# Giovannibriglia/VectorizedBayesianNetwork

Measured on AMD Instinct MI355X. Metric: posterior queries/sec (infer_posterior, n_samples=1024) at 1/2/4/8 MI355X, higher is better.
Workload: dtype f32; 1 GPU; cfg4: 64node-kde10k-mcm; queries_per_gpu=4096, global_batch=4096, n_samples=1024, n_nodes=64, engine=monte_carlo_marginalization, parallelism=query-sharded dp1, gather=False, prune_barren=False, exact_f32=False, kde_distances=mfma, walk=plan-specialised (step table compiled in with hiprtc), plan_cache_hits=1, kde_moment_nodes=16

## Files before the change

### vectorizedbayesiannetwork_amd/csrc/vbn_walk_impl.h

```cpp
#pragma once
#ifndef __HIPCC_RTC__
#include <hip/hip_runtime.h>
#include <stdint.h>
#include <math.h>
#include <stdio.h>
#include <string.h>

#include <algorithm>
#endif

#include "vbn_hip_types.h"

#ifndef INFINITY
#define INFINITY __builtin_inff()
#endif

#define WAVE 64
#define KDE_CHUNKS 16
#define KDE_MT(st) ((st).reserved[7])
#define KDE_REC_TAIL 16
#define LOG_2PI_F 1.8378770664093453f

typedef float f32x16 __attribute__((ext_vector_type(16)));
typedef _Float16 f16x8 __attribute__((ext_vector_type(8)));
typedef _Float16 f16x2 __attribute__((ext_vector_type(2)));
typedef float f32x2 __attribute__((ext_vector_type(2)));
typedef float f32x4 __attribute__((ext_vector_type(4)));

#define OFF_W2H(st) ((st).reserved[0])


__device__ __forceinline__ void wave_sync() {
  __atomic_signal_fence(__ATOMIC_SEQ_CST);
  __builtin_amdgcn_wave_barrier();
  __atomic_signal_fence(__ATOMIC_SEQ_CST);
}

__device__ __forceinline__ float relu_nan(float x) { return __int_as_float(max(__float_as_int(x), 0)); }

template <int ACT>
__device__ __forceinline__ float act_fn(float x) {
  if (ACT == VBN_ACT_RELU) return relu_nan(x);
  if (ACT == VBN_ACT_TANH) return tanhf(x);
  if (ACT == VBN_ACT_GELU) return x * 0.5f * (1.0f + erff(x * 0.70710678118654752440f));
  return x > 0.f ? x : expm1f(x);
}

#define VBN_LN2_F 0.69314718055994530942f
__device__ __forceinline__ float log_hw(float x) { return __builtin_amdgcn_logf(x) * VBN_LN2_F; }

__device__ __forceinline__ float softplus_t(float x) {
#ifdef VBN_ABL_NOSOFTPLUS
  return x;
#endif
  if (x > 20.f) return x;
  const float e = __expf(x);
  if (x < -5.f) return e * (1.f - e * (0.5f - e * (0.33333334f - e * 0.25f)));
  const float u = 1.0f + e;
  return log_hw(u) * (e * __builtin_amdgcn_rcpf(u - 1.0f));
}

__device__ __forceinline__ uint2 philox2x32(uint2 c, uint32_t k) {
#pragma unroll
  for (int r = 0; r < 10; ++r) {
    const uint64_t p = (uint64_t)0xD256D193u * c.x;
    c = make_uint2(__builtin_amdgcn_bitop3_b32((uint32_t)(p >> 32), k, c.y, 0x96), (uint32_t)p);
    k += 0x9E3779B9u;
  }
  return c;
}

__device__ __forceinline__ float u01(uint32_t x) { return (float)(x >> 8) * (1.0f / 16777216.0f); }

__device__ __forceinline__ float bm_radius(float u1) {
  return __builtin_amdgcn_sqrtf(-2.0f * log_hw(u1));
}

__device__ __forceinline__ float box_muller(uint32_t a, uint32_t b) {
  const float u1 = (float)((a >> 8) + 1u) * (1.0f / 16777216.0f);
  const float u2 = (float)(b >> 8) * (1.0f / 16777216.0f);
  return bm_radius(u1) * __builtin_amdgcn_cosf(u2);
}

struct Lane {
  const float* P;
  const int32_t* ic;
  float* vals;
  float* scr;
  const float* wb;
  int lane;
  int64_t p;
  int64_t b;
  int s;
  int iter;
  bool valid;
  bool mirror;
  bool lean;
  bool noiseless;
  bool wq;
  mutable float bm_spare;
};

// ... 1188 lines not shown
template <class ARG>
__device__ __forceinline__ int kde_scan(const float4* __restrict__ rec, const float4* __restrict__ rev, int M,
                                        int j0, int j1, float rem, float csum, ARG arg) {
  const bool back = rem > 0.5f * csum;
  const float goal = back ? csum - rem : rem;
  const float lim = back ? float_below(goal) : goal;
  const float4* __restrict__ q = back ? rev + (M - j1) : rec + j0;
  const int n = j1 - j0;
  float cs = 0.f, c0 = 0.f, c1 = 0.f, c2 = 0.f, c3 = 0.f;
  int kt = n;
  float4 a0 = q[0], a1 = q[1], a2 = q[2], a3 = q[3];
  float4 b0 = q[4], b1 = q[5], b2 = q[6], b3 = q[7];
  for (int k = 0; k < n; k += 8) {
    {
      const float e0 = cs + __builtin_amdgcn_exp2f(arg(a0));
      const float e1 = e0 + __builtin_amdgcn_exp2f(arg(a1));
      const float e2 = e1 + __builtin_amdgcn_exp2f(arg(a2));
      const float e3 = e2 + __builtin_amdgcn_exp2f(arg(a3));
      if (e3 > lim) { c0 = e0; c1 = e1; c2 = e2; c3 = e3; kt = k; break; }
      cs = e3;
    }
    a0 = q[k + 8]; a1 = q[k + 9]; a2 = q[k + 10]; a3 = q[k + 11];
    if (k + 4 >= n) break;
    {
      const float e0 = cs + __builtin_amdgcn_exp2f(arg(b0));
      const float e1 = e0 + __builtin_amdgcn_exp2f(arg(b1));
      const float e2 = e1 + __builtin_amdgcn_exp2f(arg(b2));
      const float e3 = e2 + __builtin_amdgcn_exp2f(arg(b3));
      if (e3 > lim) { c0 = e0; c1 = e1; c2 = e2; c3 = e3; kt = k + 4; break; }
      cs = e3;
    }
    b0 = q[k + 12]; b1 = q[k + 13]; b2 = q[k + 14]; b3 = q[k + 15];
  }
  (void)c3;
  const int v = c0 > lim ? 0 : (c1 > lim ? 1 : (c2 > lim ? 2 : 3));
  const int kh = kt < n ? min(kt + v, n - 1) : n - 1;
  return min(max(back ? j1 - 1 - kh : j0 + kh, 0), M - 1);
}

#define KDE_MT_HEAD 8
#define KDE_MT_GROUP 8
__device__ __forceinline__ int kde_index_moments(const float* __restrict__ T, float xb0, float ucat,
                                                 const float4* __restrict__ rec, int M, float& total) {
  const cfloat* H = CP(T);
  const float u_lo = H[0], inv_d = H[1], dlt = H[2];
  const int n_cells = __float_as_int(H[3]), nch = __float_as_int(H[4]), per = __float_as_int(H[5]);
  const float gr = rintf((xb0 - u_lo) * inv_d);
  const bool in = gr >= 0.f && gr < (float)n_cells;
  if (!__all(in)) return -1;
  const float d = xb0 - fmaf(gr, dlt, u_lo);
  const int ng = (nch + KDE_MT_GROUP - 1) / KDE_MT_GROUP;
  const float4* __restrict__ row = reinterpret_cast<const float4*>(T + KDE_MT_HEAD) + (int)gr * (nch + ng + 1);
  auto poly = [&](const float4 c) { return fmaf(fmaf(fmaf(c.w, d, c.z), d, c.y), d, c.x); };
  total = poly(row[nch + ng]);
  const double thr = (double)ucat * (double)total;
  double cum = 0.0;
  float gs = 0.f;
  int g = ng - 1;
  bool hit = false;
  for (int k = 0; k < ng; ++k) {
    gs = poly(row[nch + k]);
    const double nx = cum + (double)gs;
    if (nx > thr) { g = k; hit = true; break; }
    cum = nx;
  }
  if (!hit) cum -= (double)gs;
  const int c1 = min(nch, (g + 1) * KDE_MT_GROUP);
  int ch = c1 - 1;
  float cs = 0.f;
  hit = false;
  for (int c = g * KDE_MT_GROUP; c < c1; ++c) {
    cs = poly(row[c]);
    const double nx = cum + (double)cs;
    if (nx > thr) { ch = c; hit = true; break; }
    cum = nx;
  }
  if (!hit) cum -= (double)cs;
  const int j0 = min(M, ch * per), j1 = min(M, j0 + per);
  const float4* __restrict__ rev = rec + (((M + 15) >> 4) * 16 + KDE_REC_TAIL);
  return kde_scan(rec, rev, M, j0, j1, (float)(thr - cum), cs,
                  [&](const float4 r) { return fmaf(r.y, -1.f, fmaf(r.x, xb0, -0.f)); });
}

__device__ __forceinline__ int kde_index_mfma(const vbn_walk_args& A, const vbn_step& st, const Lane& L,
                                              float ucat, float c_p, float& lsp) {
  const int M = st.k, nf = st.aux0, lane = L.lane;
  const int cb = kde_cb(M);
  int slots[4] = {0, 0, 0, 0};
  float scl[4] = {c_p, c_p, c_p, c_p};
  for (int f = 0; f < nf; ++f) slots[f] = L.ic[st.in_off + f];
  double tot = 0.0;
  float xv[4] = {0.f, 0.f, 0.f, 0.f};
  const float negsq = kde_own(L, slots, scl, nf, xv);
  const bool pre = (st.flags & VBN_F_PRECOMP) != 0;
  const float4* __restrict__ rec = reinterpret_cast<const float4*>(L.P + st.reserved[3]) + 4;
  if (nf == 1 && KDE_MT(st) >= 0 && !(st.flags & (VBN_F_PRECOMP | VBN_F_PRE_OUT)) &&
      __all(-negsq <= KDE_FFORM_MAX)) {
    float mtot = 0.f;
    const int idx = kde_index_moments(L.P + KDE_MT(st), 2.f * xv[0], ucat, rec, M, mtot);
    if (idx >= 0) {
      if (mtot > 0.f) lsp = __logf(mtot) + negsq * VBN_LN2_F;
      wave_sync();
      return idx;
    }
  }
  float shift = 0.f;
  bool halves = false;
#ifndef VBN_ABL_NOHALVES
  float hs[KDE_CHUNKS * (KDE_NSUB - 1)];
#endif
  if (pre) {
    if (st.flags & VBN_F_PRECOMP_Q) {
      const cfloat* q = precomp_qrow(A, st, L);
      for (int ch = 0; ch < KDE_CHUNKS; ++ch) {
        const float cs = q[ch];
        L.scr[ch * WAVE + lane] = cs;
        tot += (double)cs;
      }
      shift = q[KDE_CHUNKS];
    } else {
      const float* __restrict__ q = precomp_row(A, st, L);
      for (int ch = 0; ch < KDE_CHUNKS; ++ch) {
        const float cs = q[ch];
        L.scr[ch * WAVE + lane] = cs;
        tot += (double)cs;
      }
      shift = q[KDE_CHUNKS];
    }
  } else
#ifdef VBN_ABL_NOP1
  if (true) {
    for (int ch = 0; ch < KDE_CHUNKS; ++ch) { L.scr[ch * WAVE + lane] = 1.f; tot += 1.0; }
  } else
#endif
  {
    const bf16x8* __restrict__ pa = reinterpret_cast<const bf16x8*>(L.P + st.reserved[1]) + lane;
    const bool fform = __all(-negsq <= KDE_FFORM_MAX);
    shift = fform ? 0.f : -negsq;
#ifndef VBN_ABL_NOHALVES
    float* hsp = ((st.flags & VBN_F_PRE_OUT) || (cb >> 1) < KDE_HALF_MIN) ? nullptr : hs;
    halves = hsp != nullptr;
#else
    float* hsp = nullptr;
#endif
    if (nf == 1)
      tot = kde_pass1<1, 1>(pa, cb >> 1, L, slots, scl, nf, fform, hsp);
    else if (nf == 2 && fform)
      tot = kde_pass1<1, 2>(pa, cb >> 1, L, slots, scl, nf, fform, hsp);
    else
      tot = kde_pass1<2, 2>(pa, cb >> 1, L, slots, scl, nf, fform, hsp);
  }
  const int nfr = nf;
  const float xb0 = 2.f * xv[0], xb1 = 2.f * xv[1], xb2 = 2.f * xv[2];
  if (!pre && !(tot >= (double)kde_tiny(M))) {
    halves = false;
    float amax = -INFINITY;
    for (int j = 0; j < M; ++j) amax = fmaxf(amax, kde_arg_rec(rec[j], xb0, xb1, xb2, 0.f, nfr));
    shift = amax;
    tot = 0.0;
    for (int ch = 0; ch < KDE_CHUNKS; ++ch) {
      const int j0 = min(M, ch * cb * 16), j1 = min(M, j0 + cb * 16);
      float cs = 0.f;
      for (int j = j0; j < j1; ++j)
        cs += __builtin_amdgcn_exp2f(kde_arg_rec(rec[j], xb0, xb1, xb2, 0.f, nfr) - shift);
      L.scr[ch * WAVE + lane] = cs;
      tot += (double)cs;
    }
  }
  if (tot > 0.0) lsp = __logf((float)tot) + (shift + negsq) * VBN_LN2_F;
  if (st.flags & VBN_F_PRE_OUT) {
    for (int c = 0; c < KDE_CHUNKS; ++c) vwrite(L, st.out_col + c, L.scr[c * WAVE + lane]);
    vwrite(L, st.out_col + KDE_CHUNKS, shift);
    wave_sync();
    return -1;
  }
  const double thr = (double)ucat * tot;
  double cum = 0.0;
  int ch = KDE_CHUNKS - 1;
  for (int c2 = 0; c2 < KDE_CHUNKS; ++c2) {
    const double nx = cum + (double)L.scr[c2 * WAVE + lane];
    if (nx > thr) { ch = c2; break; }
    cum = nx;
  }
  const int j0 = min(M, ch * cb * 16), j1 = min(M, j0 + cb * 16);
#ifdef VBN_ABL_NOSCAN
  wave_sync();
  return min(j0, M - 1);
#endif
  float rem = (float)(thr - cum);
  float csum = L.scr[ch * WAVE + lane];
  int jlo = j0, jhi = j1;
#ifndef VBN_ABL_NOHALVES
  if (halves) {
    const double rd = thr - cum;
    float plo = 0.f, phi = csum;
    int klo = 0, khi = KDE_NSUB;
#pragma unroll
    for (int k = 1; k < KDE_NSUB; ++k) {
      const float pk = hs[ch * (KDE_NSUB - 1) + k - 1];
      if (rd >= (double)pk) { klo = k; plo = pk; }
      else if (khi == KDE_NSUB) { khi = k; phi = pk; }
    }
    const int cb32 = cb >> 1;
    jlo = klo ? min(M, j0 + 32 * kde_sub_blocks(cb32, klo)) : j0;
    jhi = khi < KDE_NSUB ? min(M, j0 + 32 * kde_sub_blocks(cb32, khi)) : j1;
    rem = (float)(rd - (double)plo);
    csum = phi - plo;
  }
#endif
  const float4* __restrict__ rev = rec + (((M + 15) >> 4) * 16 + KDE_REC_TAIL);
  int idx;
  const float nsh = -shift;
  if (nfr == 1)
    idx = kde_scan(rec, rev, M, jlo, jhi, rem, csum,
                   [&](const float4 r) { return fmaf(r.y, -1.f, fmaf(r.x, xb0, nsh)); });
  else if (nfr == 2)
    idx = kde_scan(rec, rev, M, jlo, jhi, rem, csum, [&](const float4 r) {
      return fmaf(r.z, -1.f, fmaf(r.y, xb1, fmaf(r.x, xb0, nsh)));
    });
  else
    idx = kde_scan(rec, rev, M, jlo, jhi, rem, csum, [&](const float4 r) {
      return fmaf(r.w, -1.f, fmaf(r.z, xb2, fmaf(r.y, xb1, fmaf(r.x, xb0, nsh))));
    });
  wave_sync();
  return idx;
}

__device__ __forceinline__ bool kde_logp_mfma(const vbn_step& st, const Lane& L, bool root, float c_p,
                                              float c_y, float cy, float log_n, float& lp, float lsp) {
  const int M = st.k, dp = st.aux0, D = st.out_dim, lane = L.lane;
  const int nb32 = min((KDE_CHUNKS * kde_cb(M)) >> 1, (((M + 31) >> 5) + KDE_PF - 1) / KDE_PF * KDE_PF);
  int slots[4] = {0, 0, 0, 0};
  float scl[4] = {c_p, c_p, c_p, c_p};
  for (int f = 0; f < dp; ++f) slots[f] = L.ic[st.in_off + f];
  for (int d = 0; d < D; ++d) { slots[dp + d] = st.out_col + d; scl[dp + d] = c_y; }
  const int ny = dp + D;
  float xv[4];
  const float sq_y = -kde_own(L, slots, scl, ny, xv);
  const float sq_p = root ? 0.f : -kde_own(L, slots, scl, dp, xv);
  const bool fform = __all(sq_y <= KDE_FFORM_MAX);
  const bf16x8* __restrict__ pay = reinterpret_cast<const bf16x8*>(L.P + st.reserved[2]) + lane;
  const float sy = kde_sums_nf(pay, nb32, L, slots, scl, ny, fform);
  constexpr float LN2 = 0.69314718055994531f;
#ifndef VBN_ABL_NOLSP
  if (!root && __all(lsp == lsp)) {
    wave_sync();
    if (!(sy >= kde_tiny(M))) return false;
    lp += ((__logf(sy) - (fform ? sq_y * LN2 : 0.f)) - lsp) + cy;
    return true;
  }
#endif
  float sp = 1.f;
  if (!root) {
    const bf16x8* __restrict__ pa = reinterpret_cast<const bf16x8*>(L.P + st.reserved[1]) + lane;
    sp = kde_sums_nf(pa, nb32, L, slots, scl, dp, fform);
  }
  wave_sync();
  if (!(sy >= kde_tiny(M)) || !(sp >= kde_tiny(M))) return false;
  const float corr = fform ? (root ? sq_y : sq_y - sq_p) * LN2 : 0.f;
  lp += root ? ((__logf(sy) - corr) + cy - log_n) : (((__logf(sy) - __logf(sp)) - corr) + cy);
  return true;
}

__device__ __forceinline__ int kde_csz(int M) { return (((M + KDE_CHUNKS - 1) / KDE_CHUNKS) + 7) & ~7; }

template <int NF>
__device__ __forceinline__ float kde_arg_valu(const float (&xv)[4], const float4 r) {
#pragma clang fp contract(off)
  const float d0 = xv[0] - r.x;
  float a = d0 * d0;
  if (NF > 1) { const float d1 = xv[1] - r.y; a = fmaf(d1, d1, a); }
  if (NF > 2) { const float d2 = xv[2] - r.z; a = fmaf(d2, d2, a); }
  return -a;
}

template <int NF>
__device__ __forceinline__ int kde_index_valu(const vbn_walk_args& A, const vbn_step& st, const Lane& L,
                                              float ucat, float c_p) {
#pragma clang fp contract(off)
  const float* __restrict__ kv = L.P + st.reserved[4];
  const int M = st.k, lane = L.lane, csz = kde_csz(M);
  float xv[4] = {0.f, 0.f, 0.f, 0.f};
// ... 434 lines not shown
```

### vectorizedbayesiannetwork_amd/plan.py

```python
from __future__ import annotations

import hashlib
import math
import os
from dataclasses import dataclass
from typing import Dict, List, Optional, Sequence, Tuple

import numpy as np
import torch
import torch.nn.functional as F

from .model import BNModel, CPDRecord

KIND_ID = {"gaussian_nn": 0, "linear_gaussian": 1, "mdn": 2, "kde": 3, "softmax_nn": 4, "categorical_table": 5}
KIND_MASK_TABLE = 1024
ROLE_SKIP, ROLE_LATENT, ROLE_FIXED, ROLE_PARAMS, ROLE_SELECT, ROLE_COLLECT = 0, 1, 2, 3, 4, 5
F_LOGP, F_ROOT, F_SHARED, F_STANDARDIZE, F_CLIP, F_F32L2, F_KDE_VALU = 1, 2, 4, 8, 16, 32, 64
F_KEEP, F_LPRESET, F_BM_FIRST, F_BM_SECOND, F_MLP_GENERIC = 128, 256, 512, 1024, 2048
ACT_ID = {"relu": 0, "tanh": 1, "gelu": 2, "elu": 3}
WITHIN_ID = {"uniform": 0, "triangular": 1, "gaussian": 2}
MODE_MCM, MODE_WEIGHTED, MODE_SAMPLE, MODE_GIBBS = 0, 1, 2, 3
STEP_INTS = 32
(S_KIND, S_ROLE, S_FLAGS, S_ACT, S_NIN, S_INOFF, S_OUTCOL, S_OUTDIM, S_FIXEDCOL, S_K, S_NOUT,
 S_NODEID, S_NOISE, S_AUX0, S_AUX1, S_AUX2, S_OFF_STD, S_OFF_W1, S_OFF_W2, S_OFF_B2, S_OFF_W3,
# ... 118 lines not shown
    csz = ((m + KDE_CHUNKS - 1) // KDE_CHUNKS + 7) & ~7
    a = np.full((KDE_CHUNKS * csz, nf), 1e15, np.float32)
    a[:m] = y
    return a.reshape(-1, 8, nf).transpose(0, 2, 1)


KDE_MOMENTS = os.environ.get("VBN_KDE_MOMENTS", "1") != "0"
KDE_MT_TERMS = 4
KDE_MT_Z = 0.028
KDE_MT_CHUNKS = 64
KDE_MT_MAX_CELLS = 16384
KDE_MT_EXP_MAX = 100.0
KDE_MT_EXP_MIN = -80.0
KDE_MT_HEADER = 8


def kde_moment_cells(y: np.ndarray):
    y = np.asarray(y, np.float32).reshape(-1)
    y64 = y.astype(np.float64)
    sq = (y64 * y64).astype(np.float32).astype(np.float64)
    ymax_abs = float(np.abs(y64).max())
    span = float(y64.max() - y64.min())
    w = max(span, 2.0)
    lo, hi = 2.0 * (float(y64.min()) - w), 2.0 * (float(y64.max()) + w)
    if ymax_abs == 0.0:
        delta = hi - lo
    else:
        delta = 2.0 * KDE_MT_Z / (math.log(2.0) * ymax_abs)
    delta32 = np.float32(delta)
    lo32 = np.float32(lo)
    n = int(math.ceil((hi - lo) / float(delta32))) + 1
    if n > KDE_MT_MAX_CELLS:
        return None
    centres = kde_moment_centres(lo32, delta32, n)
    e_max = np.max(centres[:, None] * y64[None, :] - sq[None, :], axis=1)
    if e_max.max() > KDE_MT_EXP_MAX or e_max.min() < KDE_MT_EXP_MIN:
        return None
    return lo32, delta32, np.float32(1.0 / float(delta32)), n


def kde_moment_centres(lo32, delta32, n: int) -> np.ndarray:
    g = np.arange(n, dtype=np.float64)
    return (g * np.float64(delta32) + np.float64(lo32)).astype(np.float32).astype(np.float64)


def kde_moment_chunks(m: int) -> Tuple[int, int]:
    per = -(-m // KDE_MT_CHUNKS)
    return -(-m // per), per


KDE_MT_GROUP = 8


def kde_moment_rows(n_chunks: int) -> int:
    return n_chunks + -(-n_chunks // KDE_MT_GROUP) + 1


def kde_moment_table(y: np.ndarray) -> Optional[np.ndarray]:
    cells = kde_moment_cells(y)
    if cells is None:
        return None
    lo32, delta32, inv32, n = cells
    y64 = np.asarray(y, np.float32).reshape(-1).astype(np.float64)
    sq = (y64 * y64).astype(np.float32).astype(np.float64)
    m = y64.size
    nch, per = kde_moment_chunks(m)
    centres = kde_moment_centres(lo32, delta32, n)
    pw = np.stack([(math.log(2.0) * y64) ** k / math.factorial(k) for k in range(KDE_MT_TERMS)], axis=1)
    ng = -(-nch // KDE_MT_GROUP)
    tab = np.zeros((n, kde_moment_rows(nch), KDE_MT_TERMS), np.float64)
    for j0 in range(0, m, 4096):
        j1 = min(m, j0 + 4096)
        wts = np.exp2(centres[:, None] * y64[None, j0:j1] - sq[None, j0:j1])
        contrib = wts[:, :, None] * pw[None, j0:j1, :]
        chunk = np.arange(j0, j1) // per
        for c in np.unique(chunk):
            tab[:, c, :] += contrib[:, chunk == c, :].sum(axis=1)
    for g in range(ng):
        tab[:, nch + g, :] = tab[:, g * KDE_MT_GROUP:min(nch, (g + 1) * KDE_MT_GROUP), :].sum(axis=1)
    tab[:, nch + ng, :] = tab[:, :nch, :].sum(axis=1)
    head = np.zeros(KDE_MT_HEADER, np.float32)
    head[:3] = [lo32, inv32, delta32]
    head[3:6] = np.array([n, nch, per], np.int32).view(np.float32)
    return np.concatenate([head, tab.astype(np.float32).reshape(-1)])


def _np(t: torch.Tensor) -> np.ndarray:
    return t.detach().to("cpu", torch.float32).numpy()


def _pack_mlp_generic(blob: _Blob, layers, offs: Dict[str, int]) -> Dict[str, int]:
    lane = np.arange(64)
    table = [len(layers)]
    for w, b in layers:
        w, b = _np(w), _np(b)
        out, nin = w.shape
        nblk, t1 = -(-out // 32), -(-nin // 2)
        wz = np.zeros((nblk * 32, 2 * t1), np.float32)
        wz[:out, :nin] = w
        frag = np.stack([np.stack([wz[32 * k + (lane & 31), 2 * t + (lane >> 5)] for t in range(t1)])
                         for k in range(nblk)])
        bz = np.zeros(nblk * 32, np.float32)
        bz[:out] = b
        bias = np.stack([bz[32 * k + _ROWS] for k in range(nblk)])
        table += [nin, out, blob.add(frag), blob.add(bias)]
    offs["w2"] = blob.add(np.asarray(table, np.int32).view(np.float32))
    offs["n_out"] = int(_np(layers[-1][0]).shape[0])
    offs["generic"] = 1
    offs["scratch"] = offs["n_out"] + 2 * max([int(w.shape[0]) for w, _ in layers[:-1]] + [1])
    return offs


def _pack_mlp(blob: _Blob, rec: CPDRecord, standardize: bool) -> Dict[str, int]:
    layers = rec.mlp_layers()
    hidden = tuple(int(w.shape[0]) for w, _ in layers[:-1])
    offs: Dict[str, int] = {}
    if standardize:
        inv = (np.float32(1.0) / _np(rec.state["std_x"]).astype(np.float32)).astype(np.float32)
        offs["std"] = blob.add(np.concatenate([_np(rec.state["mean_x"]), inv]))
    else:
        offs["std"] = 0
    if hidden != MLP_HIDDEN:
        return _pack_mlp_generic(blob, layers, offs)
    (w1, b1), (w2, b2), (w3, b3) = [(_np(w), _np(b)) for w, b in layers]
    nin = w1.shape[1]
    t1 = (nin + 1) // 2
    w1z = np.zeros((32, 2 * t1), np.float32)
    w1z[:, :nin] = w1
    lane = np.arange(64)
    w1f = np.stack([w1z[lane & 31, 2 * t + (lane >> 5)] for t in range(t1)])
    w2f = np.zeros((16, 64), np.float32)
    for s in range(16):
        w2f[s] = w2[lane & 31, _ROWS[lane >> 5, s]]
    offs["w1"] = blob.add(w1f)
    offs["wblk"] = offs["w1"]
    offs["b2"] = blob.add(np.stack([np.stack([b[_ROWS]] * 2) for b in (b1, b2)]))
    offs["f32l2"] = int(np.abs(w2).max() > 32768.0)
    rs = float(np.abs(w1.astype(np.float64)).sum(axis=1).max()) if w1.size else 0.0
    lim = 2048.0 if str(rec.hp("activation") or "relu") == "relu" else 32768.0
    room = lim * (1.0 - 1e-3) - float(np.abs(b1.astype(np.float64)).max())
    if room <= 1.0:
        offs["zlim"] = -1.0
    else:
        offs["zlim"] = float(np.float32(min(room / rs, 3.0e38))) if rs > 0 else 3.0e38
    j = np.arange(8)
    j3 = j
    frag = np.zeros((2, 64, 8), np.float32)
    for s in range(2):
        for ln in range(64):
            frag[s, ln] = w2[ln & 31, 16 * s + 8 * (j >> 2) + 4 * (ln >> 5) + (j & 3)]
    with np.errstate(over="ignore", invalid="ignore"):
        hi = frag.astype(np.float16)
        lo = (frag - hi.astype(np.float32)).astype(np.float16)
    halfs = np.concatenate([hi, lo]).reshape(-1)
    offs["w2h"] = blob.add(halfs.view(np.float32))
    offs["w3"] = blob.add(np.concatenate([w3[:, _ROWS[0]], w3[:, _ROWS[1]]], axis=1))
    offs["b3"] = blob.add(b3)
    n_out = w3.shape[0]
    if HEAD_MFMA_MIN <= n_out <= 32 and np.abs(w3).max() <= 32768.0:
        w3p = np.zeros((32, 32), np.float32)
        w3p[:n_out] = w3
        f3 = np.zeros((2, 64, 8), np.float32)
        for s_ in range(2):
            for ln in range(64):
                f3[s_, ln] = w3p[ln & 31, 16 * s_ + 8 * (j3 >> 2) + 4 * (ln >> 5) + (j3 & 3)]
        hi3 = f3.astype(np.float16)
# ... 57 lines not shown
    scratch: int = 0


def _pack_node(blob: _Blob, rec: CPDRecord) -> NodePack:
    kind = rec.kind
    D = rec.output_dim
    root = rec.is_root
    flags = F_ROOT if root else 0
    st = rec.state
    offs: Dict[str, int] = {}
    k = n_out = aux0 = aux1 = 0
    if kind == "categorical_table":
        offs = _pack_table(blob, rec)
        k, aux0, aux1 = offs.pop("_table")
        return NodePack(kind=KIND_ID[kind], flags=flags, act=0, n_in=rec.input_dim, out_dim=D, k=k, n_out=0,
                        aux0=aux0, aux1=aux1, offs=offs, scratch=0)
    act = ACT_ID.get(str(rec.hp("activation") or "relu"), -1)
    if act < 0:
        raise ValueError(f"unknown activation {rec.hp('activation')}")
    if kind == "gaussian_nn":
        if root:
            loc = st["_loc"].view(1, 1, -1)
            scale = (F.softplus(st["_log_scale"]) + float(rec.hp("min_scale"))).view(1, 1, -1)
            std_y = st["std_y"].view(1, 1, -1)
            loc, scale = loc * std_y + st["mean_y"].view(1, 1, -1), scale * std_y
            loc, scale = loc.reshape(-1), scale.reshape(-1)
            offs["tail"] = blob.add(np.concatenate([_np(loc), _np(scale), _np(scale.log())]))
        else:
            flags |= F_STANDARDIZE
            offs.update(_pack_mlp(blob, rec, standardize=True))
            n_out = offs.pop("n_out")
            offs["tail"] = blob.add(np.concatenate([_np(st["std_y"]), _np(st["mean_y"]),
                                                    np.array([rec.hp("min_scale")], np.float32)]))
    elif kind == "linear_gaussian":
        var = st["_var"]
        scale = torch.sqrt(var.clamp(min=float(rec.hp("min_scale")) ** 2))
        w = st["_weight"]
        offs["tail"] = blob.add(np.concatenate([_np(w.t().contiguous()).reshape(-1), _np(st["_bias"]),
                                                _np(scale), _np(torch.log(scale))]))
    elif kind == "mdn":
        k = int(rec.hp("n_components"))
        if root:
            pi = torch.softmax(st["_logits"], dim=-1).clamp_min(1e-5)
            pi = pi / pi.sum(dim=-1, keepdim=True).clamp_min(1e-12)
            scale = F.softplus(st["_log_scale"]) + float(rec.hp("min_scale"))
            log_scale = torch.log(scale)
            offs["tail"] = blob.add(np.concatenate([
                _np(pi), _np(torch.log(pi)), _np(st["_loc"]).reshape(-1), _np(scale).reshape(-1),
                _np(log_scale).reshape(-1), _np(torch.exp(2 * log_scale)).reshape(-1),
                _np(torch.softmax(st["_logits"], dim=-1))]))
        else:
            offs.update(_pack_mlp(blob, rec, standardize=False))
            n_out = offs.pop("n_out")
            if n_out != k * (2 * D) + k:
                raise ValueError("mdn head width mismatch")
            offs["tail"] = blob.add(np.array([rec.hp("min_scale")], np.float32))
    elif kind == "kde":
        pts_p = rec.extra["parents"].float()
        pts_y = rec.extra["targets"].float()
        m = int(pts_y.shape[0])
        dp = int(pts_p.shape[1]) if pts_p.dim() == 2 else 0
        if m == 0:
            raise RuntimeError("KDECPD is not fitted yet.")
        bw = float(rec.hp("bandwidth"))
        pbw = rec.hp("parent_bandwidth")
        pbw = bw if pbw is None else float(pbw)
        min_scale = float(rec.hp("min_scale"))
        s_p = max(pbw, 1e-3) + min_scale
        s_y = max(bw, 1e-3) + min_scale
        noise_scale = max(bw, 1e-3) + min_scale
        cy = -0.5 * D * (math.log(2 * math.pi) + 2 * math.log(s_y))
        c_p = np.float32(_KDE_C / s_p)
        c_y = np.float32(_KDE_C / s_y)
        offs["tail"] = blob.add(np.array([1.0 / np.float32(s_p), 1.0 / np.float32(s_y),
                                          noise_scale, cy, math.log(float(m)), c_p, c_y, 0], np.float32))
        if 1 <= dp <= 3:
            offs["kq"] = blob.add(_kde_pack_b32(_np(pts_p) * c_p))
            offs["kr"] = blob.add(_kde_pack([_np(pts_p) * c_p], records=True))
            offs["kv"] = blob.add(_kde_pack_valu(_np(pts_p) * c_p))
            if dp == 1 and KDE_MOMENTS:
                mt = kde_moment_table((_np(pts_p) * c_p).reshape(-1))
                if mt is not None:
                    offs["kmt"] = blob.add(mt)
        if dp + D <= 4:
            feats = np.concatenate(([_np(pts_p).reshape(m, -1) * c_p] if dp else [])
                                   + [_np(pts_y).reshape(m, -1) * c_y], axis=1)
            offs["kqy"] = blob.add(_kde_pack_b32(feats))
        stride = dp + D
        stride += (-stride) % 2 if stride > 1 else 0
        recs = np.zeros((m, stride), np.float32)
        if dp:
            recs[:, :dp] = _np(pts_p)
        recs[:, dp:dp + D] = _np(pts_y)
        offs["pts"] = blob.add(recs)
        k, aux0, aux1 = m, dp, stride
    elif kind == "softmax_nn":
        if str(rec.hp("mode_when_not_discrete") or "binned") != "binned":
            raise NotImplementedError("softmax_nn mode_when_not_discrete != 'binned'")
        if not bool(st["_bins_ready"]):
            raise RuntimeError("Bins not initialized. Call fit(...) before sampling.")
        k = int(rec.hp("n_classes"))
        aux0 = WITHIN_ID[str(rec.hp("within_bin"))]
        disc = st["_is_discrete"].bool()
        if D > 31:
            raise NotImplementedError("softmax_nn with more than 31 output dims")
        aux1 = int(sum(1 << d for d in range(D) if bool(disc[d])))
        if bool(rec.hp("within_bin_clip")):
            flags |= F_CLIP
        mbw = float(rec.hp("min_bin_width"))
        offs["tail"] = blob.add(np.concatenate([
            _np(st["_bin_edges"]).reshape(-1), _np(st["_sample_values"]).reshape(-1),
            _np(st["_class_values"]).reshape(-1),
            np.array([rec.hp("within_bin_scale"), mbw, mbw ** 2, 0.0], np.float32)]))
        if root:
            if bool(st["_root_ready"]):
                tab = torch.log_softmax(st["_root_log_probs"].view(D, k) / 1.0, dim=-1)
            else:
                tab = st["_logits"].view(D, k) / 1.0
            offs["pts"] = blob.add(_np(tab))
        else:
            offs.update(_pack_mlp(blob, rec, standardize=False))
            n_out = offs.pop("n_out")
    else:
        raise ValueError(kind)
    if offs.pop("generic", 0):
        flags |= F_MLP_GENERIC
    if offs.pop("f32l2", 0):
        flags |= F_F32L2
    scratch = offs.pop("scratch", n_out)
    return NodePack(kind=KIND_ID[kind], flags=flags, act=max(act, 0), n_in=rec.input_dim,
                    out_dim=D, k=k, n_out=n_out, aux0=aux0, aux1=aux1, offs=offs, scratch=scratch)


class PackedModel:

    def __init__(self, model: BNModel, device: torch.device):
        self.model = model
        self.device = torch.device(device)
        blob = _Blob()
        blob.add(np.zeros(4, np.float32))
        self.nodes: Dict[str, NodePack] = {}
        if len(model.topo) >= MAX_NODES:
            raise NotImplementedError(f"{len(model.topo)} nodes: the walk keys RNG streams for < {MAX_NODES}")
        for node in model.topo:
            if model.out_dim(node) >= MAX_NODE_DIMS:
                raise NotImplementedError(f"node {node}: {model.out_dim(node)} dims (max {MAX_NODE_DIMS - 1})")
            rec = model.cpds[node]
            expect = sum(model.out_dim(p) for p in model.parents[node])
            if rec.input_dim != expect:
                raise ValueError(f"node {node}: CPD input_dim {rec.input_dim} != parents width {expect}")
            self.nodes[node] = _pack_node(blob, rec)
        host = blob.finish()
        self.tabular = all(p.kind == KIND_ID["categorical_table"] for p in self.nodes.values())
        if self.tabular and host.size % WBLK_CHUNK:
            host = np.concatenate([host, np.zeros((-host.size) % WBLK_CHUNK, np.float32)])
        self.params = torch.from_numpy(host).to(self.device)
        self.node_id = {n: i for i, n in enumerate(model.topo)}
        self.max_out = max([p.scratch for p in self.nodes.values()] + [1])
        self.has_kde = any(p.kind == KIND_ID["kde"] for p in self.nodes.values())
        self.dmax = max(model.out_dim(n) for n in model.topo)


@dataclass
class QueryPlan:
    steps: torch.Tensor
    in_cols: torch.Tensor
# ... 129 lines not shown
    slot_of: Dict[str, int] = {}
    release: Dict[int, List[str]] = {}
    for i, n in enumerate(order):
        d = width(n)
        base = None
        if d == 1 and free:
            free.sort()
            base = free.pop(0)
        elif d > 1:
            fs = sorted(free)
            for j in range(len(fs) - d + 1):
                if fs[j + d - 1] - fs[j] == d - 1:
                    base = fs[j]
                    for q in range(d):
                        free.remove(base + q)
                    break
        if base is None:
            base = n_slots
            n_slots += d
        slot_of[n] = base
        release.setdefault(last[n], []).append(n)
        for m in release.pop(i, []):
            if m != n or last[n] == i:
                free.extend(range(slot_of[m], slot_of[m] + width(m)))
    fixed_nodes = [n for n in order if n in fixed_s]
    fixed_col = {}
    c = 0
    for n in fixed_nodes:
        fixed_col[n] = c
        c += model.out_dim(n)
    noise_nodes = [n for n in order if n in latent_s]
    noise_idx = {n: i for i, n in enumerate(noise_nodes)}
    steps = np.zeros((len(order), STEP_INTS), np.int32)
    in_cols: List[int] = []
    for i, n in enumerate(order):
        npk = packed.nodes[n]
        row = steps[i]
        row[S_KIND] = npk.kind
        row[S_ROLE] = ROLE_PARAMS if n in params_s else (ROLE_LATENT if n in latent_s else ROLE_FIXED)
        fl = npk.flags
        if n in logp_s:
            fl |= F_LOGP
        if shared_roots and (npk.flags & F_ROOT):
            fl |= F_SHARED
        if exact_f32:
            fl |= F_F32L2
        if kde_valu and npk.kind == KIND_ID["kde"]:
            fl |= F_KDE_VALU
        if n in pre_s:
            fl |= F_PRE_OUT
        if n in clamp_s and n in fixed_s:
            fl |= F_CLAMP_EV
        row[S_FLAGS] = fl
        row[S_ACT] = npk.act
        row[S_NIN] = npk.n_in
        row[S_INOFF] = len(in_cols)
        if reads[n]:
            for p in model.parents[n]:
                in_cols.extend(range(slot_of[p], slot_of[p] + model.out_dim(p)))
        row[S_OUTCOL] = slot_of[n]
        row[S_OUTDIM] = npk.out_dim
        row[S_FIXEDCOL] = fixed_col.get(n, 0)
        row[S_K] = npk.k
        row[S_NOUT] = npk.n_out
        row[S_NODEID] = packed.node_id[n]
        row[S_NOISE] = noise_idx.get(n, 0)
        row[S_AUX0] = npk.aux0
        row[S_AUX1] = npk.aux1
        for key, idx in (("std", S_OFF_STD), ("w1", S_OFF_W1), ("w2", S_OFF_W2), ("b2", S_OFF_B2),
                         ("w3", S_OFF_W3), ("b3", S_OFF_B3), ("tail", S_OFF_TAIL), ("pts", S_OFF_PTS),
                         ("w2h", S_OFF_W2H)):
            row[idx] = npk.offs.get(key, 0)
        row[S_OFF_KQ] = npk.offs.get("kq", -1)
        if "zlim" in npk.offs:
            row[S_OFF_KQ] = np.float32(npk.offs["zlim"]).view(np.int32)
        row[S_OFF_KQY] = npk.offs.get("kqy", -1)
        if "w3h" in npk.offs:
            row[S_OFF_KQY] = npk.offs["w3h"]
            fl |= F_HEAD_MFMA
            row[S_FLAGS] = fl
        row[S_OFF_KR] = npk.offs.get("kr", -1)
        row[S_OFF_KV] = npk.offs.get("kv", -1)
        row[S_RES7] = npk.offs.get("kmt", -1)
        if "wblk" in npk.offs and (n in latent_s or n in logp_s or n in params_s):
            row[S_WBLK_OFF] = npk.offs["wblk"]
            row[S_WBLK_LEN] = npk.offs["wblk_len"]
    out_cols: List[int] = []
    for n in out_nodes:
        out_cols.extend(range(slot_of[n], slot_of[n] + width(n)))
    dev = packed.device

    def t(a):
        a = np.asarray(a, np.int32).reshape(-1) if len(a) else np.zeros(1, np.int32)
        return torch.from_numpy(np.ascontiguousarray(a)).to(dev)

    _pair_normals(steps)
    kind_mask = 0
    for n in order:
        if n in latent_s or n in logp_s or n in params_s:
            npk = packed.nodes[n]
            kind_mask |= 1 << npk.kind
            if npk.n_out and npk.act != ACT_ID["relu"]:
                kind_mask |= 32
            if npk.flags & F_MLP_GENERIC:
                kind_mask |= 512
    tabular = bool(getattr(packed, "tabular", False))
    wbuf = int(steps[:, S_WBLK_LEN].max()) if len(order) else 0
    if tabular:
        kind_mask = KIND_MASK_TABLE
        wbuf = int(packed.params.numel())
        read_by = {p for n in order if reads[n] for p in model.parents[n]}
        table_check = [(n, fixed_col[n], n in clamp_s) for n in fixed_nodes
                       if n in logp_s or n in read_by or n in set(out_nodes)]
        cv_offs: List[int] = []
        for n in out_nodes:
            npk = packed.nodes[n]
            if n in params_s:
                cv_offs.extend([-1] * width(n))
            else:
                cv_offs.extend(npk.offs["w3"] + dd * npk.aux1 for dd in range(npk.out_dim))
    max_out = max([packed.nodes[n].scratch for n in order] + [1])
    if any(packed.nodes[n].kind == KIND_ID["kde"] for n in order):
        max_out = max(max_out, KDE_CHUNKS)
    steps_t = torch.from_numpy(steps).to(dev) if len(order) else torch.zeros(1, STEP_INTS, dtype=torch.int32, device=dev)
    steps_t._vbn_wblk_max = int(steps[:, S_WBLK_LEN].max()) if len(order) else 0
    ic_host = np.asarray(in_cols, np.int32).reshape(-1)
    steps_t._vbn_host = (steps.copy(), ic_host.copy(),
                         hashlib.sha1(steps.tobytes() + b"|" + ic_host.tobytes()).hexdigest())
    return QueryPlan(
        steps=steps_t,
        in_cols=t(in_cols), out_cols=t(out_cols), n_steps=len(order), n_slots=max(n_slots, 1),
        max_out=max_out, fixed_nodes=fixed_nodes, fixed_ld=max(c, 1), noise_nodes=noise_nodes,
        out_nodes=list(out_nodes), mode=mode, slot_of=slot_of, kind_mask=kind_mask, order=list(order),
        wbuf=wbuf, tabular=tabular, table_out_cols=t(out_cols + cv_offs) if tabular else None,
        table_check=table_check if tabular else None)


def _pair_normals(steps: np.ndarray) -> None:
    gauss = (KIND_ID["gaussian_nn"], KIND_ID["linear_gaussian"], KIND_ID["mdn"], KIND_ID["kde"])
    pending = -1
    for i in range(len(steps)):
        r = steps[i]
        if r[S_ROLE] != ROLE_LATENT or r[S_KIND] not in gauss or r[S_OUTDIM] != 1:
            continue
        if pending >= 0 and (steps[pending][S_FLAGS] & F_SHARED) == (r[S_FLAGS] & F_SHARED):
            steps[pending][S_FLAGS] |= F_BM_FIRST
            r[S_FLAGS] |= F_BM_SECOND
            pending = -1
        else:
            pending = i


@dataclass
class GibbsPlan:
    init: QueryPlan
    steps: torch.Tensor
    n_steps: int
    latent: List[str]
    target: str
    n_noise: int
    in_cols: torch.Tensor
    kind_mask: int
    wbuf: int = 0


def build_gibbs_plan(packed: PackedModel, *, latent: Sequence[str], fixed: Sequence[str], target: str,
# ... 350 lines not shown
```

Baseline: 55580 queries/s.

## Add 2D moment-table lookup for two-parent KDE chunk sums

Result: faster. 59770 queries/s, median of 6 (+7.5%).

```diff
diff --git a/vectorizedbayesiannetwork_amd/csrc/vbn_walk_impl.h b/vectorizedbayesiannetwork_amd/csrc/vbn_walk_impl.h
--- a/vectorizedbayesiannetwork_amd/csrc/vbn_walk_impl.h
+++ b/vectorizedbayesiannetwork_amd/csrc/vbn_walk_impl.h
@@ -18,6 +18,7 @@
 #define WAVE 64
 #define KDE_CHUNKS 16
 #define KDE_MT(st) ((st).reserved[7])
+#define KDE_MT2(st) ((st).off_w1)
 #define KDE_REC_TAIL 16
 #define LOG_2PI_F 1.8378770664093453f
 
@@ -1372,6 +1373,60 @@
                   [&](const float4 r) { return fmaf(r.y, -1.f, fmaf(r.x, xb0, -0.f)); });
 }
 
+#define KDE_MT2_HEAD 16
+#define KDE_MT2_K 9
+#define KDE_MT2_ROW4 12
+struct KdeMt2 {
+  const float4* cell;
+  float d0, d1;
+};
+
+__device__ __forceinline__ float kde_mt2_row(const float4* __restrict__ row, float d0, float d1) {
+  float4 v = row[0];
+  int i = 0;
+  auto next = [&]() {
+    const int k = i & 3;
+    if (i && !k) v = row[i >> 2];
+    ++i;
+    return k == 0 ? v.x : (k == 1 ? v.y : (k == 2 ? v.z : v.w));
+  };
+  float s = next();
+#pragma unroll
+  for (int a = KDE_MT2_K - 2; a >= 0; --a) {
+    float p = next();
+#pragma unroll
+    for (int b = KDE_MT2_K - 2 - a; b >= 0; --b) p = fmaf(p, d1, next());
+    s = fmaf(s, d0, p);
+  }
+  return s;
+}
+
+__device__ __noinline__ float kde_mt2_row_call(const float4* __restrict__ row, float d0, float d1) {
+  return kde_mt2_row(row, d0, d1);
+}
+
+__device__ __forceinline__ bool kde_index_moments2(const float* __restrict__ T, float u0, float u1, const Lane& L,
+                                                   bool halves, double& tot, KdeMt2& m) {
+  const cfloat* H = CP(T);
+  const float g0 = rintf((u0 - H[0]) * H[1]), g1 = rintf((u1 - H[4]) * H[5]);
+  const int n0 = __float_as_int(H[3]), n1 = __float_as_int(H[7]);
+  const bool in = g0 >= 0.f && g0 < (float)n0 && g1 >= 0.f && g1 < (float)n1;
+  if (!__all(in)) return false;
+  m.d0 = u0 - fmaf(g0, H[2], H[0]);
+  m.d1 = u1 - fmaf(g1, H[6], H[4]);
+  const int rows = halves ? 2 * KDE_CHUNKS : KDE_CHUNKS;
+  m.cell = reinterpret_cast<const float4*>(T + KDE_MT2_HEAD) + ((int)g0 * n1 + (int)g1) * (rows * KDE_MT2_ROW4);
+  double t = 0.0;
+#pragma unroll 1
+  for (int ch = 0; ch < KDE_CHUNKS; ++ch) {
+    const float cs = kde_mt2_row(m.cell + ch * KDE_MT2_ROW4, m.d0, m.d1);
+    L.scr[ch * WAVE + L.lane] = cs;
+    t += (double)cs;
+  }
+  tot = t;
+  return true;
+}
+
 __device__ __forceinline__ int kde_index_mfma(const vbn_walk_args& A, const vbn_step& st, const Lane& L,
                                               float ucat, float c_p, float& lsp) {
   const int M = st.k, nf = st.aux0, lane = L.lane;
@@ -1396,6 +1451,23 @@
   }
   float shift = 0.f;
   bool halves = false;
+  bool tab2 = false;
+  KdeMt2 mt2 = {nullptr, 0.f, 0.f};
+  if (nf == 2 && KDE_MT2(st) >= 0 && !(st.flags & (VBN_F_PRECOMP | VBN_F_PRE_OUT)) &&
+      __all(-negsq <= KDE_FFORM_MAX)) {
+#ifndef VBN_ABL_NOHALVES
+    const bool h2 = KDE_NSUB == 2 && (cb >> 1) >= KDE_HALF_MIN;
+#else
+    const bool h2 = false;
+#endif
+    double t2 = 0.0;
+    if (kde_index_moments2(L.P + KDE_MT2(st), 2.f * xv[0], 2.f * xv[1], L, (cb >> 1) >= KDE_HALF_MIN, t2, mt2) &&
+        __all(t2 >= (double)kde_tiny(M))) {
+      tab2 = true;
+      halves = h2;
+      tot = t2;
+    }
+  }
 #ifndef VBN_ABL_NOHALVES
   float hs[KDE_CHUNKS * (KDE_NSUB - 1)];
 #endif
@@ -1417,7 +1489,7 @@
       }
       shift = q[KDE_CHUNKS];
     }
-  } else
+  } else if (!tab2)
 #ifdef VBN_ABL_NOP1
   if (true) {
     for (int ch = 0; ch < KDE_CHUNKS; ++ch) { L.scr[ch * WAVE + lane] = 1.f; tot += 1.0; }
@@ -1487,7 +1559,8 @@
     int klo = 0, khi = KDE_NSUB;
 #pragma unroll
     for (int k = 1; k < KDE_NSUB; ++k) {
-      const float pk = hs[ch * (KDE_NSUB - 1) + k - 1];
+      const float pk = tab2 ? kde_mt2_row_call(mt2.cell + (KDE_CHUNKS + ch) * KDE_MT2_ROW4, mt2.d0, mt2.d1)
+                            : hs[ch * (KDE_NSUB - 1) + k - 1];
       if (rd >= (double)pk) { klo = k; plo = pk; }
       else if (khi == KDE_NSUB) { khi = k; phi = pk; }
     }
diff --git a/vectorizedbayesiannetwork_amd/plan.py b/vectorizedbayesiannetwork_amd/plan.py
--- a/vectorizedbayesiannetwork_amd/plan.py
+++ b/vectorizedbayesiannetwork_amd/plan.py
@@ -224,6 +224,95 @@
     head = np.zeros(KDE_MT_HEADER, np.float32)
     head[:3] = [lo32, inv32, delta32]
     head[3:6] = np.array([n, nch, per], np.int32).view(np.float32)
+    return np.concatenate([head, tab.astype(np.float32).reshape(-1)])
+
+
+KDE_MOMENTS2 = os.environ.get("VBN_KDE_MOMENTS2", "1") != "0"
+KDE_MT2_Z = 0.5
+KDE_MT2_K = 9
+KDE_MT2_COEFS = KDE_MT2_K * (KDE_MT2_K + 1) // 2
+KDE_MT2_ROW = (KDE_MT2_COEFS + 3) & ~3
+KDE_MT2_HEADER = 16
+KDE_MT2_MAX_BYTES = 32 << 20
+KDE_MT2_MARGINS = (2.0, 1.5, 1.0)
+KDE_HALF_MIN = 16
+
+
+def kde_moment2_order(k: int = KDE_MT2_K) -> List[Tuple[int, int]]:
+    return [(a, b) for a in range(k - 1, -1, -1) for b in range(k - 1 - a, -1, -1)]
+
+
+def kde_moment2_geometry(m: int) -> Tuple[int, int, bool]:
+    cb = _kde_cb(m)
+    cb32 = cb // 2
+    return 16 * cb, 32 * ((cb32 // 2) & ~1), cb32 >= KDE_HALF_MIN
+
+
+def kde_moment2_cells(y: np.ndarray, z: float = KDE_MT2_Z, w: float = KDE_MT2_MARGINS[0]):
+    y64 = np.asarray(y, np.float32).reshape(-1, 2).astype(np.float64)
+    out = []
+    for f in range(2):
+        c = y64[:, f]
+        lo, hi = 2.0 * (float(c.min()) - w), 2.0 * (float(c.max()) + w)
+        amax = float(np.abs(c).max())
+        delta32 = np.float32(hi - lo if amax == 0.0 else z / (math.log(2.0) * amax))
+        lo32 = np.float32(lo)
+        n = int(math.ceil((hi - lo) / float(delta32))) + 1
+        out.append((lo32, delta32, np.float32(1.0 / float(delta32)), n))
+    return out
+
+
+def kde_moment_table2(y: np.ndarray, z: float = KDE_MT2_Z, k: int = KDE_MT2_K) -> Optional[np.ndarray]:
+    y32 = np.asarray(y, np.float32).reshape(-1, 2)
+    m = y32.shape[0]
+    per, half, halves = kde_moment2_geometry(m)
+    rows = KDE_CHUNKS * (2 if halves else 1)
+    order = kde_moment2_order(k)
+    rowf = (len(order) + 3) & ~3
+    for w in KDE_MT2_MARGINS:
+        (lo0, dl0, inv0, n0), (lo1, dl1, inv1, n1) = kde_moment2_cells(y32, z, w)
+        if n0 * n1 * rows * rowf * 4 <= KDE_MT2_MAX_BYTES:
+            break
+    else:
+        return None
+    y64 = y32.astype(np.float64)
+    sq = (y64 ** 2).sum(axis=1).astype(np.float32).astype(np.float64)
+    c0, c1 = kde_moment_centres(lo0, dl0, n0), kde_moment_centres(lo1, dl1, n1)
+    ly = math.log(2.0) * y64
+    pw = np.stack([ly[:, 0] ** a * ly[:, 1] ** b / (math.factorial(a) * math.factorial(b)) for a, b in order], axis=1)
+    tab = np.zeros((n0 * n1, rows, rowf), np.float64)
+    w_max = np.zeros(n0 * n1)
+    blk = max(256, (1 << 22) // (n0 * n1))
+
+    def seg_sum(j0, j1):
+        acc = np.zeros((n0 * n1, len(order)))
+        for i0 in range(j0, j1, blk):
+            i1 = min(j1, i0 + blk)
+            e0 = np.exp2(c0[:, None] * y64[None, i0:i1, 0] - sq[None, i0:i1])
+            e1 = np.exp2(c1[:, None] * y64[None, i0:i1, 1])
+            wts = (e0[:, None, :] * e1[None, :, :]).reshape(n0 * n1, i1 - i0)
+            np.maximum(w_max, wts.max(axis=1), out=w_max)
+            acc += wts @ pw[i0:i1]
+        return acc
+
+    for c in range(KDE_CHUNKS):
+        j0, j1 = min(m, c * per), min(m, (c + 1) * per)
+        if j0 >= j1:
+            continue
+        jh = min(j1, j0 + half) if halves else j0
+        first = seg_sum(j0, jh) if jh > j0 else 0.0
+        tab[:, c, :len(order)] = first + (seg_sum(jh, j1) if j1 > jh else 0.0)
+        if halves:
+            tab[:, KDE_CHUNKS + c, :len(order)] = first
+    with np.errstate(divide="ignore"):
+        e_max = np.log2(w_max)
+    if not (e_max.max() <= KDE_MT_EXP_MAX and e_max.min() >= KDE_MT_EXP_MIN):
+        return None
+    head = np.zeros(KDE_MT2_HEADER, np.float32)
+    head[0:3] = [lo0, inv0, dl0]
+    head[4:7] = [lo1, inv1, dl1]
+    head[[3, 7]] = np.array([n0, n1], np.int32).view(np.float32)
+    head[8:11] = np.array([rows, rowf, k], np.int32).view(np.float32)
     return np.concatenate([head, tab.astype(np.float32).reshape(-1)])
 
 
@@ -447,6 +536,10 @@
                 mt = kde_moment_table((_np(pts_p) * c_p).reshape(-1))
                 if mt is not None:
                     offs["kmt"] = blob.add(mt)
+            if dp == 2 and KDE_MOMENTS2:
+                mt = kde_moment_table2(_np(pts_p) * c_p)
+                if mt is not None:
+                    offs["kmt2"] = blob.add(mt)
         if dp + D <= 4:
             feats = np.concatenate(([_np(pts_p).reshape(m, -1) * c_p] if dp else [])
                                    + [_np(pts_y).reshape(m, -1) * c_y], axis=1)
@@ -742,6 +835,8 @@
         row[S_OFF_KR] = npk.offs.get("kr", -1)
         row[S_OFF_KV] = npk.offs.get("kv", -1)
         row[S_RES7] = npk.offs.get("kmt", -1)
+        if npk.kind == KIND_ID["kde"]:
+            row[S_OFF_W1] = npk.offs.get("kmt2", -1)
         if "wblk" in npk.offs and (n in latent_s or n in logp_s or n in params_s):
             row[S_WBLK_OFF] = npk.offs["wblk"]
             row[S_WBLK_LEN] = npk.offs["wblk_len"]
```
